# AlirezaMoseni/Distributed-Optimization-and-Learning

Measured on AMD Instinct MI355X. Metric: consensus rounds/sec at 8192 agents x 1M params (1/8 GPU) + % of HBM peak, higher is better.
Workload: dtype f32

## Files before the change

distributed-optimization-and-learning_amd/csrc/mlp_step.hip:

```cpp
#include <hip/hip_runtime.h>
#include <stdint.h>
#include <stdio.h>
#include <stdlib.h>
#include <math.h>
#include <type_traits>

#include "../../include/dol_hip.h"
#include "dol_common.h"

namespace {

typedef float f4 __attribute__((ext_vector_type(4)));
typedef float f32x16 __attribute__((ext_vector_type(16)));

constexpr int kWaves = 4;
constexpr int kThreads = 64 * kWaves;
constexpr int kMaxB = 64, kMaxH = 256, kMaxC = 32;

struct MlpArgs {
  float* W; int64_t ldw;
  float* G; int64_t ldg;
  float* M; int64_t ldm;
  const float* theta;
  const float* A; int64_t lda;
  const float* X; int64_t ldxa, ldxb;
  const int64_t* Y; int64_t ldya;
  float* loss;
  int B, d, h, c;
  float neg_lr, mom, rho;
  int mode;
  int update;
  int f1_keep;
  int dw1_reverse;
  int stagger, stagger_lo, stagger_hi, stagger_step;
#ifdef DOL_MLP_TRACE
  long long* trace;
#endif
};

#ifdef DOL_MLP_TRACE
#define DOL_TRACE(i) \
  if (threadIdx.x == 0 && a.trace) a.trace[int64_t(blockIdx.x) * 8 + (i)] = wall_clock64();
#else
#define DOL_TRACE(i)
#endif

template <int N, int UPD, bool TH, bool AL>
struct ParamBatch {
  float w[N], m[N], th[N], al[N];

  template <class Idx>
  __device__ __forceinline__ void load(const MlpArgs& a, const float* wrow, const float* mrow, const float* arow,
                                       Idx idx) {
#pragma unroll
    for (int i = 0; i < N; ++i) {
      if constexpr (UPD > 0 || TH) w[i] = wrow[idx(i)];
      if constexpr (UPD == 3) m[i] = mrow[idx(i)];
      if constexpr (TH) th[i] = a.theta[idx(i)];
      if constexpr (AL) al[i] = arow[idx(i)];
    }
  }

  template <class Idx, class Ok>
  __device__ __forceinline__ void commit(const MlpArgs& a, float* wrow, float* grow, float* mrow, const float (&g)[N],
                                         Idx idx, Ok ok) {
#pragma unroll
    for (int i = 0; i < N; ++i) {
      float gg = g[i];
      if constexpr (TH) {
        float t = a.rho * (w[i] - th[i]);
        if constexpr (AL) t = al[i] + t;
        gg = gg + t;
      }
      float dd = gg;
      if constexpr (UPD == 2) {
        m[i] = gg;
      } else if constexpr (UPD == 3) {
        m[i] = m[i] * a.mom + gg;
        dd = m[i];
      }
      if (!ok(i)) continue;
      if (grow) grow[idx(i)] = gg;
      if constexpr (UPD > 0) __builtin_nontemporal_store(__builtin_fmaf(a.neg_lr, dd, w[i]), wrow + idx(i));
      if constexpr (UPD >= 2) __builtin_nontemporal_store(m[i], mrow + idx(i));
    }
  }
};

#define DOL_GPTR(p) ((const __attribute__((address_space(1))) void*)(p))
#define DOL_LPTR(p) ((__attribute__((address_space(3))) void*)(p))

__device__ __forceinline__ void wait_vmcnt(int n) {
  switch (n) {
#define DOL_VMC(N) case N: asm volatile("s_waitcnt vmcnt(" #N ")" ::: "memory"); break;
#define DOL_VMC8(N) DOL_VMC(N) DOL_VMC(N + 1) DOL_VMC(N + 2) DOL_VMC(N + 3) DOL_VMC(N + 4) DOL_VMC(N + 5) DOL_VMC(N + 6) DOL_VMC(N + 7)
    DOL_VMC8(0) DOL_VMC8(8) DOL_VMC8(16) DOL_VMC8(24) DOL_VMC8(32) DOL_VMC8(40) DOL_VMC8(48) DOL_VMC8(56)
#undef DOL_VMC8
#undef DOL_VMC
    default: asm volatile("s_waitcnt vmcnt(0)" ::: "memory"); break;
  }
}

template <int N, class Src, class Dst>
__device__ __forceinline__ void lds_fill(int n, Src src, Dst dst) {
  const int t = threadIdx.x;
  for (int o0 = 0; o0 < n; o0 += N * kThreads) {
    float v[N];
#pragma unroll
    for (int i = 0; i < N; ++i) {
      const int o = o0 + i * kThreads + t;
      v[i] = src(o < n ? o : 0);
    }
#pragma unroll
    for (int i = 0; i < N; ++i) {
      const int o = o0 + i * kThreads + t;
      if (o < n) dst(o, v[i]);
    }
  }
}

__device__ __forceinline__ void lds_barrier() {
  asm volatile("s_waitcnt lgkmcnt(0)" ::: "memory");
  __builtin_amdgcn_s_barrier();
  asm volatile("" ::: "memory");
}

constexpr int kStages = 3;

inline int64_t fwd_union_floats(int B, int h, int c) {
  const int64_t staging = int64_t(kStages) * (h + 32 * ((B + 31) / 32)) * 32;
  const int64_t post = int64_t(B) * (h + 4) + int64_t(c) * (h + 4) + int64_t(B) * c;
  return staging > post ? staging : post;
}

using rsrc_t = __amdgpu_buffer_rsrc_t;
constexpr uint32_t kOOB = 0x80000000u;

__device__ __forceinline__ rsrc_t make_rsrc(const float* p, int64_t nbytes) {
  return __builtin_amdgcn_make_buffer_rsrc(const_cast<float*>(p), 0, static_cast<int>(nbytes), 0x00020000);
}
__device__ __forceinline__ float bload(rsrc_t r, uint32_t voff, uint32_t soff) {
  return __builtin_bit_cast(float, __builtin_amdgcn_raw_buffer_load_b32(r, static_cast<int>(voff), static_cast<int>(soff), 0));
}
__device__ __forceinline__ void bstore_nt(rsrc_t r, uint32_t voff, uint32_t soff, float v) {
  __builtin_amdgcn_raw_buffer_store_b32(__builtin_bit_cast(uint32_t, v), r, static_cast<int>(voff), static_cast<int>(soff), 2);
}

template <int NT, int UPD, bool TH, bool AL>
__device__ __forceinline__ void mlp_fwd_body(MlpArgs a, float* __restrict__ ws) {
  constexpr int NS = kStages;
  if (a.stagger > 0) {
    const int bx = int(blockIdx.x);
    if (bx >= a.stagger_lo && bx < a.stagger_hi && (bx - a.stagger_lo) % a.stagger_step == 0)
      for (int i = 0; i < a.stagger; ++i) __builtin_amdgcn_s_sleep(127);
  }
  extern __shared__ __attribute__((aligned(16))) float lds[];
  const int B = a.B, d = a.d, h = a.h, c = a.c;
  const int hp = h + 4;
  const int64_t stg_rows = h + 32 * ((B + 31) / 32);
  float* Hs = lds;
  float* W2s = Hs + B * hp;
  float* Zs = W2s + c * hp;
  const int64_t stg_f = stg_rows * (32 * NS);
  const int64_t post_f = int64_t(B) * (h + 4) + int64_t(c) * (h + 4) + int64_t(B) * c;
  float* b1s = lds + (stg_f > post_f ? stg_f : post_f);
  float* b2s = b1s + h;
  float* ls = b2s + c;
  int* ys = reinterpret_cast<int*>(ls + B);

  const int agent = blockIdx.x;
  const int t = threadIdx.x, lane = t & 63;
  const int wave = __builtin_amdgcn_readfirstlane(t >> 6);
  const int li = lane & 31, hh = lane >> 5;
  float* wrow = a.W + int64_t(agent) * a.ldw;
  float* grow = a.G ? a.G + int64_t(agent) * a.ldg : nullptr;
  float* mrow = a.M ? a.M + int64_t(agent) * a.ldm : nullptr;
  const float* arow = a.A ? a.A + int64_t(agent) * a.lda : nullptr;
  const float* xa = a.X + int64_t(agent) * a.ldxa;
  const int64_t oW1 = 0, ob1 = int64_t(h) * d, oW2 = ob1 + h, ob2 = oW2 + int64_t(c) * h;

  DOL_TRACE(0)
  auto ok_w2 = [&](int i) { return i * kThreads + t < c * h; };
  auto idx_w2 = [&](int i) { return oW2 + (ok_w2(i) ? i * kThreads + t : 0); };
  auto ok_b1 = [&](int) { return t < h; };
  auto idx_b1 = [&](int) { return ob1 + (t < h ? t : 0); };
  auto ok_b2 = [&](int) { return t < c; };
  auto idx_b2 = [&](int) { return ob2 + (t < c ? t : 0); };
  ParamBatch<8, UPD, TH, AL> pw2;
  ParamBatch<1, UPD, TH, AL> pb1, pb2;
  auto load_small = [&] {
    pw2.load(a, wrow, mrow, arow, idx_w2);
    pb1.load(a, wrow, mrow, arow, idx_b1);
    pb2.load(a, wrow, mrow, arow, idx_b2);
  };
  load_small();
  if (t < c) b2s[t] = wrow[ob2 + t];
  if (t < B) ys[t] = static_cast<int>(a.Y[int64_t(agent) * a.ldya + t]);
  for (int i = t; i < h; i += kThreads) b1s[i] = wrow[ob1 + i];
  lds_barrier();
  float* wsa = ws + int64_t(agent) * B * h;
  const bool w2_in_regs = (UPD > 0 || TH) && c * h <= 8 * kThreads;
  const int nht = h / 32, nbt = (B + 31) / 32;
  const int Bp = 32 * nbt, rows = h + Bp;
  const int ipw = rows / 32;
  const int nk = (d + 31) / 32;
  float* stg = lds;
  const rsrc_t rsX = make_rsrc(xa, (int64_t(B - 1) * a.ldxb + d) * 4);
  (void)rsX;
  auto issue = [&](int kc, const float* top, int i0) {
    float* st = stg + (kc % NS) * rows * 32;
    for (int i = i0; i < ipw; ++i) {
      const int ins = wave + kWaves * i;
      const int r = 8 * ins + (lane >> 3);
      const int ch = (lane & 7) ^ (lane >> 3);
      int k = kc * 32 + 4 * ch;
      k = k < d ? k : 0;
      const float* src = (r < h) ? top + oW1 + int64_t(r) * d + k
                                 : xa + int64_t(min(r - h, B - 1)) * a.ldxb + k;
      if (a.f1_keep)
        __builtin_amdgcn_global_load_lds(DOL_GPTR(src), DOL_LPTR(st + ins * 256), 16, 0, 0);
      else
        __builtin_amdgcn_global_load_lds(DOL_GPTR(src), DOL_LPTR(st + ins * 256), 16, 0, 2);
    }
  };
  f32x16 acc[NT];
#pragma unroll
  for (int u = 0; u < NT; ++u)
#pragma unroll
    for (int r = 0; r < 16; ++r) acc[u][r] = 0.f;
  for (int s0 = 0; s0 < NS - 1 && s0 < nk; ++s0) issue(s0, wrow, 0);
  auto f1_chunk = [&](int kc) __attribute__((always_inline)) {
    wait_vmcnt(min(NS - 2, nk - 1 - kc) * ipw);
    __builtin_amdgcn_s_barrier();
    const float* st = stg + (kc % NS) * rows * 32;
    if (kc == nk - 1 && (d & 31)) {
      for (int i = 0; i < ipw; ++i) {
        const int ins = wave + kWaves * i;
        if (kc * 32 + 4 * ((lane & 7) ^ (lane >> 3)) >= d)
          *reinterpret_cast<f4*>(const_cast<float*>(st) + ins * 256 + lane * 4) = f4{0.f, 0.f, 0.f, 0.f};
      }
      lds_barrier();
    }
    if (kc + NS - 1 < nk) issue(kc + NS - 1, wrow, 0);
#pragma unroll
    for (int u = 0; u < NT; ++u) {
      const int tile = wave + kWaves * u;
      if (tile < nht * nbt) {
        const int ht = tile % nht, bt = tile / nht;
        const float* ar = st + (32 * ht + li) * 32;
        const float* xr = st + (h + 32 * bt + li) * 32;
#pragma unroll
        for (int j = 0; j < 4; ++j) {
          const int pos = ((4 * hh + j) ^ (li & 7)) * 4;
          const f4 av = *reinterpret_cast<const f4*>(ar + pos);
          const f4 xv = *reinterpret_cast<const f4*>(xr + pos);
#pragma unroll
          for (int q = 0; q < 4; ++q) acc[u] = __builtin_amdgcn_mfma_f32_32x32x2f32(av[q], xv[q], acc[u], 0, 0, 0);
        }
      }
    }
  };
  for (int kc = 0; kc < nk; ++kc) f1_chunk(kc);
  lds_barrier();
#pragma unroll
  for (int u = 0; u < NT; ++u) {
    const int tile = wave + kWaves * u;
    if (tile < nht * nbt) {
      const int ht = tile % nht, bt = tile / nht;
      const int brow = 32 * bt + li;
      if (brow < B) {
#pragma unroll
        for (int r = 0; r < 16; ++r) {
          const int hr = 32 * ht + (r & 3) + 8 * (r >> 2) + 4 * hh;
          const float z = acc[u][r] + b1s[hr];
          Hs[brow * hp + hr] = (z > 0.0f || z != z) ? z : 0.0f;
        }
      }
    }
  }
  if (w2_in_regs) {
#pragma unroll
    for (int i = 0; i < 8; ++i)
      if (ok_w2(i)) W2s[((i * kThreads + t) / h) * hp + (i * kThreads + t) % h] = pw2.w[i];
  } else {
    lds_fill<8>(c * h, [&](int o) { return wrow[oW2 + o]; }, [&](int o, float v) { W2s[(o / h) * hp + o % h] = v; });
  }
  lds_barrier();

  DOL_TRACE(1)
  for (int o = t; o < B * c; o += kThreads) {
    const int b = o / c, j = o % c;
    float s0 = 0.0f, s1 = 0.0f, s2 = 0.0f, s3 = 0.0f;
#pragma unroll 8
    for (int k = 0; k < h; k += 4) {
      const f4 hv = *reinterpret_cast<const f4*>(Hs + b * hp + k);
      const f4 wv = *reinterpret_cast<const f4*>(W2s + j * hp + k);
      s0 = s0 + hv.x * wv.x;
      s1 = s1 + hv.y * wv.y;
      s2 = s2 + hv.z * wv.z;
      s3 = s3 + hv.w * wv.w;
    }
    Zs[o] = ((s0 + s1) + (s2 + s3)) + b2s[j];
  }
  lds_barrier();

  if (t < B) {
    float* z = Zs + t * c;
    float m = z[0];
    for (int j = 1; j < c; ++j) m = fmaxf(m, z[j]);
    float s = 0.0f;
    for (int j = 0; j < c; ++j) s = s + expf(z[j] - m);
    const float lse = m + logf(s);
    const int y = ys[t];
    const bool yok = y >= 0 && y < c;
    ls[t] = yok ? lse - z[yok ? y : 0] : __builtin_nanf("");
    const float invB = 1.0f / static_cast<float>(B);
    for (int j = 0; j < c; ++j) z[j] = (expf(z[j] - lse) - (j == y ? 1.0f : 0.0f)) * invB;
  }
  lds_barrier();
  if (t == 0 && a.loss) {
    float s = 0.0f;
#pragma unroll 8
    for (int b = 0; b < B; ++b) s = s + ls[b];
    a.loss[agent] = s / static_cast<float>(B);
  }

  DOL_TRACE(2)
  for (int o0 = 0; o0 < c * h; o0 += 8 * kThreads) {
    ParamBatch<8, UPD, TH, AL> pb;
    float g[8];
    auto ok = [&](int i) { return o0 + i * kThreads + t < c * h; };
    auto idx = [&](int i) { return oW2 + (ok(i) ? o0 + i * kThreads + t : 0); };
    if (o0 > 0) pb.load(a, wrow, mrow, arow, idx);
    if (kThreads % h == 0) {
      const int k = t % h;
      int jj[8];
#pragma unroll
      for (int i = 0; i < 8; ++i) {
        jj[i] = ok(i) ? (o0 + i * kThreads + t) / h : 0;
        g[i] = 0.0f;
      }
#pragma unroll 4
      for (int b = 0; b < B; ++b) {
        const float hv = Hs[b * hp + k];
        const float* zr = Zs + b * c;
#pragma unroll
        for (int i = 0; i < 8; ++i) g[i] = g[i] + zr[jj[i]] * hv;
      }
    } else {
#pragma unroll
      for (int i = 0; i < 8; ++i) {
        const int o = ok(i) ? o0 + i * kThreads + t : 0;
        const int j = o / h, k = o % h;
        float s = 0.0f;
        for (int b = 0; b < B; ++b) s = s + Zs[b * c + j] * Hs[b * hp + k];
        g[i] = s;
      }
    }
    if (o0 == 0) pw2.commit(a, wrow, grow, mrow, g, idx, ok);
    else pb.commit(a, wrow, grow, mrow, g, idx, ok);
  }
  DOL_TRACE(5)
  if (t < 64) {
    float g[1];
    const int j = t < c ? t : 0;
    float s = 0.0f;
#pragma unroll 8
    for (int b = 0; b < B; ++b) s = s + Zs[b * c + j];
    g[0] = s;
    pb2.commit(a, wrow, grow, mrow, g, idx_b2, ok_b2);
  }
  lds_barrier();
  DOL_TRACE(6)

  if (kThreads % h == 0 && B * h <= 16 * kThreads) {
    const int k = t % h, b0 = t / h, bs = kThreads / h;
    float sm[16];
#pragma unroll
    for (int m = 0; m < 16; ++m) sm[m] = 0.0f;
    for (int j = 0; j < c; ++j) {
      const float w2 = W2s[j * hp + k];
#pragma unroll
      for (int m = 0; m < 16; ++m) {
        const int b = b0 + m * bs;
        sm[m] = sm[m] + Zs[min(b, B - 1) * c + j] * w2;
      }
    }
#pragma unroll
    for (int m = 0; m < 16; ++m) {
      const int b = b0 + m * bs;
      if (b < B) {
        float* hv = Hs + b * hp + k;
        *hv = (*hv > 0.0f) ? sm[m] : 0.0f;
      }
    }
  } else {
#pragma unroll 4
    for (int o = t; o < B * h; o += kThreads) {
      const int b = o / h, k = o % h;
      float s = 0.0f;
      for (int j = 0; j < c; ++j) s = s + Zs[b * c + j] * W2s[j * hp + k];
      float* hv = Hs + b * hp + k;
      *hv = (*hv > 0.0f) ? s : 0.0f;
    }
  }
  lds_barrier();
  DOL_TRACE(7)

  {
    float g[1];
    float s = 0.0f;
    if (t < h)
#pragma unroll 8
      for (int b = 0; b < B; ++b) s = s + Hs[b * hp + t];
    g[0] = s;
    pb1.commit(a, wrow, grow, mrow, g, idx_b1, ok_b1);
  }

  for (int o = t; o < B * h; o += kThreads) wsa[o] = Hs[(o / h) * hp + (o % h)];
  DOL_TRACE(3)
}

template <int NT, int UPD, bool TH, bool AL>
__global__ __launch_bounds__(kThreads) void mlp_fwd_kernel(MlpArgs a, float* __restrict__ ws) {
  mlp_fwd_body<NT, UPD, TH, AL>(a, ws);
}

template <int KS, int UPD, bool TH, bool AL>
__device__ __forceinline__ void mlp_dw1_body(MlpArgs a, const float* __restrict__ ws, int n_agents) {
  const int B = a.B, d = a.d, h = a.h, c = a.c;
  const int ndt = (d + 31) / 32;
  const uint32_t bx = blockIdx.x, l = bx >> 3;
  const int dt = static_cast<int>(l % uint32_t(ndt));
  uint32_t lg = l / uint32_t(ndt);
  if (a.dw1_reverse) lg = uint32_t((n_agents + 7) / 8) - 1 - lg;
  const int agent = static_cast<int>(lg * 8 + (bx & 7));
  if (agent >= n_agents) return;
  const int lane = threadIdx.x & 63;
  const int wave = __builtin_amdgcn_readfirstlane(threadIdx.x >> 6);
  const int li = lane & 31, hh = lane >> 5;
  const int64_t P = int64_t(h) * d + h + int64_t(c) * h + c;
  const rsrc_t rW = make_rsrc(a.W + int64_t(agent) * a.ldw, P * 4);
  const rsrc_t rM = make_rsrc(UPD == 3 || UPD == 2 ? a.M + int64_t(agent) * a.ldm : a.W, P * 4);
  const rsrc_t rG = make_rsrc(a.G ? a.G + int64_t(agent) * a.ldg : a.W, a.G ? P * 4 : 0);
  const rsrc_t rT = make_rsrc(TH ? a.theta : a.W, TH ? P * 4 : 0);
  const rsrc_t rA = make_rsrc(AL ? a.A + int64_t(agent) * a.lda : a.W, AL ? P * 4 : 0);
  const rsrc_t rX = make_rsrc(a.X + int64_t(agent) * a.ldxa, (int64_t(B - 1) * a.ldxb + d) * 4);
  const rsrc_t rZ = make_rsrc(ws + int64_t(agent) * B * h, int64_t(B) * h * 4);
  const int col = 32 * dt + li;
  const bool cok = col < d;
  float xv[KS];
#pragma unroll
  for (int s = 0; s < KS; ++s) {
    const int b = 2 * s + hh;
    xv[s] = bload(rX, (b < B && cok) ? uint32_t((b * a.ldxb + col) * 4) : kOOB, 0);
  }
  for (int ht = wave; ht < h / 32; ht += kWaves) {
    float av[KS];
#pragma unroll
    for (int s = 0; s < KS; ++s) {
      const int b = 2 * s + hh;
      av[s] = bload(rZ, b < B ? uint32_t((b * h + 32 * ht + li) * 4) : kOOB, 0);
    }
    const uint32_t pv = cok ? uint32_t(((32 * ht + 4 * hh) * d + col) * 4) : kOOB;
    auto so = [&](int r) { return uint32_t(((r & 3) + 8 * (r >> 2)) * d * 4); };
    float w[16], m[16], th[16], al[16];
#pragma unroll
    for (int r = 0; r < 16; ++r) {
      if constexpr (UPD > 0 || TH) w[r] = bload(rW, pv, so(r));
      if constexpr (UPD == 3) m[r] = bload(rM, pv, so(r));
      if constexpr (TH) th[r] = bload(rT, pv, so(r));
      if constexpr (AL) al[r] = bload(rA, pv, so(r));
    }
    __builtin_amdgcn_sched_barrier(0);
    f32x16 acc;
#pragma unroll
    for (int r = 0; r < 16; ++r) acc[r] = 0.f;
    f32x16 acc1 = acc;
#pragma unroll
    for (int s = 0; s < KS; s += 2) {
      acc = __builtin_amdgcn_mfma_f32_32x32x2f32(av[s], xv[s], acc, 0, 0, 0);
      acc1 = __builtin_amdgcn_mfma_f32_32x32x2f32(av[s + 1], xv[s + 1], acc1, 0, 0, 0);
    }
    acc += acc1;
#pragma unroll
    for (int r = 0; r < 16; ++r) {
      float gg = acc[r];
      if constexpr (TH) {
        float t = a.rho * (w[r] - th[r]);
        if constexpr (AL) t = al[r] + t;
        gg = gg + t;
      }
      float dd = gg;
      if constexpr (UPD == 2) {
        m[r] = gg;
      } else if constexpr (UPD == 3) {
        m[r] = m[r] * a.mom + gg;
        dd = m[r];
      }
      if (a.G) bstore_nt(rG, pv, so(r), gg);
      if constexpr (UPD > 0) bstore_nt(rW, pv, so(r), __builtin_fmaf(a.neg_lr, dd, w[r]));
      if constexpr (UPD >= 2) bstore_nt(rM, pv, so(r), m[r]);
    }
  }
}

template <int KS, int UPD, bool TH, bool AL>
__global__ __launch_bounds__(kThreads) void mlp_dw1_kernel(MlpArgs a, const float* __restrict__ ws, int n_agents) {
  mlp_dw1_body<KS, UPD, TH, AL>(a, ws, n_agents);
}

}

extern "C" int64_t dol_mlp_step_workspace_bytes(int32_t n_agents, int32_t B, int32_t h) {
  if (n_agents <= 0 || B <= 0 || h <= 0 || B > kMaxB || h > kMaxH) return 0;
  return int64_t(n_agents) * B * h * int64_t(sizeof(float));
}

extern "C" int64_t dol_mlp_step_lds_bytes(int32_t B, int32_t h, int32_t c) {
  if (B <= 0 || h <= 0 || c <= 0 || B > kMaxB || h > kMaxH || c > kMaxC) return 0;
  return sizeof(float) * (fwd_union_floats(B, h, c) + h + c + B) + sizeof(int) * int64_t(B);
}

extern "C" int dol_mlp_step_f32(float* w, int64_t ldw, float* grad, int64_t ldg, float* mom, int64_t ldm,
                                const float* theta, const float* alpha, int64_t lda, const float* X,
                                int64_t ldx_agent, int64_t ldx_row, const int64_t* labels, int64_t ldy_agent,
                                float* loss, int32_t n_agents, int32_t B, int32_t d, int32_t h, int32_t c,
                                float lr, float momentum, float rho, int first_step, int update,
                                void* work, hipStream_t s) {
  DOL_DIMS_OK("dol_mlp_step_f32", ldw, ldg, ldm, lda, ldx_agent, ldx_row, ldy_agent);
  using dol::fail;
  if (n_agents < 0) return fail(DOL_EINVAL, "dol_mlp_step_f32: negative agent count");
  if (n_agents == 0) { dol::g_err[0] = '\0'; return DOL_OK; }
  if (B < 1 || B > kMaxB) return fail(DOL_EINVAL, "dol_mlp_step_f32: batch %d outside [1, %d]", B, kMaxB);
  if (h < 32 || h > kMaxH || h % 32) return fail(DOL_EINVAL, "dol_mlp_step_f32: hidden %d must be a multiple of 32 in [32, %d]", h, kMaxH);
  if (c < 1 || c > kMaxC) return fail(DOL_EINVAL, "dol_mlp_step_f32: classes %d outside [1, %d]", c, kMaxC);
  if (d < 4 || d % 4) return fail(DOL_EINVAL, "dol_mlp_step_f32: input dim %d must be a positive multiple of 4", d);
  if (!w || !X || !labels || !work) return fail(DOL_EINVAL, "dol_mlp_step_f32: null w / X / labels / work");
  const int64_t P = int64_t(h) * d + h + int64_t(c) * h + c;
  if (ldw < P || (grad && ldg < P) || (mom && ldm < P) || (alpha && lda < P))
    return fail(DOL_EINVAL, "dol_mlp_step_f32: ld < P (%lld)", (long long)P);
  if (ldx_row < d || ldx_agent < int64_t(B - 1) * ldx_row + d || ldy_agent < B)
    return fail(DOL_EINVAL, "dol_mlp_step_f32: X / labels strides too small");
  if ((reinterpret_cast<uintptr_t>(w) & 15) || ldw % 4 || (reinterpret_cast<uintptr_t>(X) & 15) || ldx_row % 4 ||
      ldx_agent % 4)
    return fail(DOL_EINVAL, "dol_mlp_step_f32: w and X rows must be 16-byte aligned");
  if (alpha && !theta) return fail(DOL_EINVAL, "dol_mlp_step_f32: alpha without theta");
  const int mode = (momentum == 0.0f) ? 0 : (first_step ? 1 : 2);
  if (update && mode != 0 && !mom) return fail(DOL_EINVAL, "dol_mlp_step_f32: momentum needs the mom buffer");
  if (!update && !grad) return fail(DOL_EINVAL, "dol_mlp_step_f32: update=0 needs a grad buffer to write");
  MlpArgs a{w, ldw, grad, ldg, mom, ldm, theta, alpha, lda, X, ldx_agent, ldx_row, labels, ldy_agent, loss,
            B, d, h, c, -lr, momentum, rho, update ? mode : 0, update ? 1 : 0};
  static const int f1_keep = [] { const char* e = getenv("DOL_MLP_F1_KEEP"); return e ? atoi(e) : 1; }();
  static const int dw1_rev = [] { const char* e = getenv("DOL_MLP_DW1_REVERSE"); return e ? atoi(e) : 1; }();
  a.f1_keep = f1_keep;
  a.dw1_reverse = dw1_rev;
  {
    static const int n_cu = [] {
      int dev = 0, cu = 0;
      if (hipGetDevice(&dev) != hipSuccess ||
          hipDeviceGetAttribute(&cu, hipDeviceAttributeMultiprocessorCount, dev) != hipSuccess)
        cu = 0;
      return cu;
    }();
    const char* e = getenv("DOL_MLP_FWD_STAGGER");
    int cnt = (n_cu > 0 && n_agents >= 4 * n_cu) ? 6 : 0, mode = 1;
    if (e && sscanf(e, "%d,%d", &cnt, &mode) < 1) cnt = 0;
    if (cnt > 0 && n_cu > 0) {
      a.stagger = cnt;
      a.stagger_lo = mode == 2 ? 1 : n_cu;
      a.stagger_hi = 2 * n_cu;
      a.stagger_step = mode == 2 ? 2 : 1;
    }
  }
  const size_t lds = static_cast<size_t>(dol_mlp_step_lds_bytes(B, h, c));
  if (lds > 160 * 1024) return fail(DOL_EINVAL, "dol_mlp_step_f32: %zu B of LDS per agent exceeds 160 KiB", lds);
  const dim3 grid(static_cast<unsigned>(n_agents)), block(kThreads);
  const int upd = update ? mode + 1 : 0;
  float* ws = static_cast<float*>(work);
  const int64_t n_blk2 = int64_t((d + 31) / 32) * ((int64_t(n_agents) + 7) / 8 * 8);
  if (n_blk2 > (int64_t(1) << 31) - 1) return fail(DOL_EINVAL, "dol_mlp_step_f32: too many W1 tiles for one launch");
  const dim3 grid2(static_cast<unsigned>(n_blk2));
  auto go = [&](auto ks, auto upd_c, auto th, auto al) {
    constexpr int KS = decltype(ks)::value, U = decltype(upd_c)::value;
    constexpr bool TH = decltype(th)::value, AL = decltype(al)::value;
    auto fwd = [&](auto kern) {
      if (lds > 65536)
        (void)hipFuncSetAttribute(reinterpret_cast<const void*>(kern), hipFuncAttributeMaxDynamicSharedMemorySize,
                                  static_cast<int>(lds));
      hipLaunchKernelGGL(kern, grid, block, lds, s, a, ws);
    };
    if (h * ((B + 31) / 32) <= 128) fwd(mlp_fwd_kernel<1, U, TH, AL>);
    else fwd(mlp_fwd_kernel<4, U, TH, AL>);
    hipLaunchKernelGGL((mlp_dw1_kernel<KS, U, TH, AL>), grid2, block, 0, s, a, ws, n_agents);
  };
  auto by_upd = [&](auto ks, auto th, auto al) {
    using std::integral_constant;
    switch (upd) {
      case 0: go(ks, integral_constant<int, 0>{}, th, al); break;
      case 1: go(ks, integral_constant<int, 1>{}, th, al); break;
      case 2: go(ks, integral_constant<int, 2>{}, th, al); break;
      default: go(ks, integral_constant<int, 3>{}, th, al); break;
    }
  };
  using K16 = std::integral_constant<int, 16>;
  using K32 = std::integral_constant<int, 32>;
  using T = std::true_type;
  using F = std::false_type;
  if (B <= 32) {
    if (!theta) by_upd(K16{}, F{}, F{});
    else if (!alpha) by_upd(K16{}, T{}, F{});
    else by_upd(K16{}, T{}, T{});
  } else {
    if (!theta) by_upd(K32{}, F{}, F{});
    else if (!alpha) by_upd(K32{}, T{}, F{});
    else by_upd(K32{}, T{}, T{});
  }
  return dol::check_launch("dol_mlp_step_f32");
}
```

Baseline: 92.62.

## Move MLP second-layer forward and backward matmuls onto MFMA 32x32x2 f32

Replaces the scalar LDS dot-product loops for the layer-2 logits, the W2 gradient and the hidden-layer backprop with MFMA 32x32x2 f32 tiles split across waves. Per-wave partial logits go to a new LDS scratch buffer, and a separate pass reduces them and computes the softmax with wave shuffles instead of one thread per row. The W2 gradient and dH are computed in one fused pass, with the workspace write merged into it. LDS buffers are padded to 32 rows/classes, which increases LDS use and may lower occupancy. The code assumes c<=32 and B<=64.

```diff
diff --git a/distributed-optimization-and-learning_amd/csrc/mlp_step.hip b/distributed-optimization-and-learning_amd/csrc/mlp_step.hip
--- a/distributed-optimization-and-learning_amd/csrc/mlp_step.hip
+++ b/distributed-optimization-and-learning_amd/csrc/mlp_step.hip
@@ -127,9 +127,14 @@
 
 constexpr int kStages = 3;
 
+constexpr int kCp = 32;
+constexpr int kZp = 33;
+
 inline int64_t fwd_union_floats(int B, int h, int c) {
-  const int64_t staging = int64_t(kStages) * (h + 32 * ((B + 31) / 32)) * 32;
-  const int64_t post = int64_t(B) * (h + 4) + int64_t(c) * (h + 4) + int64_t(B) * c;
+  (void)c;
+  const int64_t Bp = 32 * ((B + 31) / 32);
+  const int64_t staging = int64_t(kStages) * (h + Bp) * 32;
+  const int64_t post = Bp * (h + 4) + int64_t(kCp) * (h + 4) + Bp * kZp + int64_t(kWaves) * Bp * 32;
   return staging > post ? staging : post;
 }
 
@@ -158,11 +163,14 @@
   const int B = a.B, d = a.d, h = a.h, c = a.c;
   const int hp = h + 4;
   const int64_t stg_rows = h + 32 * ((B + 31) / 32);
+  const int Bpad = 32 * ((B + 31) / 32);
   float* Hs = lds;
-  float* W2s = Hs + B * hp;
-  float* Zs = W2s + c * hp;
+  float* W2s = Hs + Bpad * hp;
+  float* Zs = W2s + kCp * hp;
+  float* Ps = Zs + Bpad * kZp;
   const int64_t stg_f = stg_rows * (32 * NS);
-  const int64_t post_f = int64_t(B) * (h + 4) + int64_t(c) * (h + 4) + int64_t(B) * c;
+  const int64_t post_f = int64_t(Bpad) * (h + 4) + int64_t(kCp) * (h + 4) + int64_t(Bpad) * kZp +
+                         int64_t(kWaves) * Bpad * 32;
   float* b1s = lds + (stg_f > post_f ? stg_f : post_f);
   float* b2s = b1s + h;
   float* ls = b2s + c;
@@ -285,128 +293,152 @@
   } else {
     lds_fill<8>(c * h, [&](int o) { return wrow[oW2 + o]; }, [&](int o, float v) { W2s[(o / h) * hp + o % h] = v; });
   }
+  for (int o = B * hp + t; o < Bpad * hp; o += kThreads) Hs[o] = 0.0f;
+  for (int o = c * hp + t; o < kCp * hp; o += kThreads) W2s[o] = 0.0f;
   lds_barrier();
 
   DOL_TRACE(1)
-  for (int o = t; o < B * c; o += kThreads) {
-    const int b = o / c, j = o % c;
-    float s0 = 0.0f, s1 = 0.0f, s2 = 0.0f, s3 = 0.0f;
-#pragma unroll 8
-    for (int k = 0; k < h; k += 4) {
-      const f4 hv = *reinterpret_cast<const f4*>(Hs + b * hp + k);
-      const f4 wv = *reinterpret_cast<const f4*>(W2s + j * hp + k);
-      s0 = s0 + hv.x * wv.x;
-      s1 = s1 + hv.y * wv.y;
-      s2 = s2 + hv.z * wv.z;
-      s3 = s3 + hv.w * wv.w;
-    }
-    Zs[o] = ((s0 + s1) + (s2 + s3)) + b2s[j];
+  auto rrow = [&](int r) { return (r & 3) + 8 * (r >> 2) + 4 * hh; };
+  {
+    f32x16 z2[2];
+#pragma unroll
+    for (int bt = 0; bt < 2; ++bt)
+#pragma unroll
+      for (int r = 0; r < 16; ++r) z2[bt][r] = 0.f;
+    for (int ht = wave; ht < nht; ht += kWaves) {
+      const int k0 = 32 * ht + 4 * hh;
+#pragma unroll
+      for (int jj = 0; jj < 4; ++jj) {
+        const f4 wv = *reinterpret_cast<const f4*>(W2s + li * hp + k0 + 8 * jj);
+#pragma unroll
+        for (int bt = 0; bt < 2; ++bt) {
+          if (bt < nbt) {
+            const f4 hv = *reinterpret_cast<const f4*>(Hs + (32 * bt + li) * hp + k0 + 8 * jj);
+#pragma unroll
+            for (int q = 0; q < 4; ++q) z2[bt] = __builtin_amdgcn_mfma_f32_32x32x2f32(hv[q], wv[q], z2[bt], 0, 0, 0);
+          }
+        }
+      }
+    }
+#pragma unroll
+    for (int bt = 0; bt < 2; ++bt)
+      if (bt < nbt)
+#pragma unroll
+        for (int r = 0; r < 16; ++r) Ps[(wave * Bpad + 32 * bt + rrow(r)) * 32 + li] = z2[bt][r];
   }
   lds_barrier();
 
-  if (t < B) {
-    float* z = Zs + t * c;
-    float m = z[0];
-    for (int j = 1; j < c; ++j) m = fmaxf(m, z[j]);
-    float s = 0.0f;
-    for (int j = 0; j < c; ++j) s = s + expf(z[j] - m);
-    const float lse = m + logf(s);
-    const int y = ys[t];
-    const bool yok = y >= 0 && y < c;
-    ls[t] = yok ? lse - z[yok ? y : 0] : __builtin_nanf("");
+  {
     const float invB = 1.0f / static_cast<float>(B);
-    for (int j = 0; j < c; ++j) z[j] = (expf(z[j] - lse) - (j == y ? 1.0f : 0.0f)) * invB;
+    const int tile = Bpad * 32;
+    for (int o = t; o < tile; o += kThreads) {
+      const int b = o >> 5, j = o & 31;
+      const bool live = j < c, bok = b < B;
+      float z = ((Ps[o] + Ps[tile + o]) + Ps[2 * tile + o]) + Ps[3 * tile + o];
+      z = z + b2s[live ? j : 0];
+      float m = live ? z : -INFINITY;
+#pragma unroll
+      for (int x = 16; x > 0; x >>= 1) m = fmaxf(m, __shfl_xor(m, x));
+      float s = live ? expf(z - m) : 0.0f;
+#pragma unroll
+      for (int x = 16; x > 0; x >>= 1) s = s + __shfl_xor(s, x);
+      const float lse = m + logf(s);
+      const int y = ys[bok ? b : B - 1];
+      const bool yok = y >= 0 && y < c;
+      const float zy = __shfl(z, (lane & 32) | (yok ? y : 0));
+      if (j == 0 && bok) ls[b] = yok ? lse - zy : __builtin_nanf("");
+      Zs[b * kZp + j] = (live && bok) ? (expf(z - lse) - (j == y ? 1.0f : 0.0f)) * invB : 0.0f;
+    }
   }
   lds_barrier();
-  if (t == 0 && a.loss) {
-    float s = 0.0f;
-#pragma unroll 8
-    for (int b = 0; b < B; ++b) s = s + ls[b];
-    a.loss[agent] = s / static_cast<float>(B);
-  }
 
   DOL_TRACE(2)
-  for (int o0 = 0; o0 < c * h; o0 += 8 * kThreads) {
-    ParamBatch<8, UPD, TH, AL> pb;
-    float g[8];
-    auto ok = [&](int i) { return o0 + i * kThreads + t < c * h; };
-    auto idx = [&](int i) { return oW2 + (ok(i) ? o0 + i * kThreads + t : 0); };
-    if (o0 > 0) pb.load(a, wrow, mrow, arow, idx);
-    if (kThreads % h == 0) {
-      const int k = t % h;
-      int jj[8];
+  {
+    const int nsb = (B + 1) / 2, nsc = (c + 1) / 2;
+    for (int ht = wave; ht < nht; ht += kWaves) {
+      const int kcol = 32 * ht + li;
+      f32x16 gw, dz[2];
+#pragma unroll
+      for (int r = 0; r < 16; ++r) gw[r] = dz[0][r] = dz[1][r] = 0.f;
+      for (int s0 = 0; s0 < nsb; s0 += 8) {
+        float za[8], hb[8];
+#pragma unroll
+        for (int u = 0; u < 8; ++u) {
+          za[u] = Zs[(2 * (s0 + u) + hh) * kZp + li];
+          hb[u] = Hs[(2 * (s0 + u) + hh) * hp + kcol];
+        }
+#pragma unroll
+        for (int u = 0; u < 8; ++u) gw = __builtin_amdgcn_mfma_f32_32x32x2f32(za[u], hb[u], gw, 0, 0, 0);
+      }
+      for (int s0 = 0; s0 < nsc; s0 += 4) {
+        float w2[4], za[2][4];
+#pragma unroll
+        for (int u = 0; u < 4; ++u) {
+          w2[u] = W2s[(2 * (s0 + u) + hh) * hp + kcol];
+#pragma unroll
+          for (int bt = 0; bt < 2; ++bt) za[bt][u] = Zs[(32 * (bt < nbt ? bt : 0) + li) * kZp + 2 * (s0 + u) + hh];
+        }
+#pragma unroll
+        for (int u = 0; u < 4; ++u)
+#pragma unroll
+          for (int bt = 0; bt < 2; ++bt)
+            if (bt < nbt) dz[bt] = __builtin_amdgcn_mfma_f32_32x32x2f32(za[bt][u], w2[u], dz[bt], 0, 0, 0);
+      }
+#pragma unroll
+      for (int bt = 0; bt < 2; ++bt) {
+        if (bt < nbt) {
+#pragma unroll
+          for (int r = 0; r < 16; ++r) {
+            const int b = 32 * bt + rrow(r);
+            if (b < B) {
+              float* hv = Hs + b * hp + kcol;
+              const float v = (*hv > 0.0f) ? dz[bt][r] : 0.0f;
+              *hv = v;
+              wsa[b * h + kcol] = v;
+            }
+          }
+        }
+      }
+#pragma unroll
+      for (int r = 0; r < 16; ++r) W2s[rrow(r) * hp + kcol] = gw[r];
+    }
+  }
+  lds_barrier();
+  DOL_TRACE(5)
+
+  {
+    const int dj = kThreads / h, dk = kThreads % h;
+    int j = t / h, k = t % h;
+    for (int o0 = 0; o0 < c * h; o0 += 8 * kThreads) {
+      ParamBatch<8, UPD, TH, AL> pb;
+      float g[8];
+      auto ok = [&](int i) { return o0 + i * kThreads + t < c * h; };
+      auto idx = [&](int i) { return oW2 + (ok(i) ? o0 + i * kThreads + t : 0); };
+      if (o0 > 0) pb.load(a, wrow, mrow, arow, idx);
 #pragma unroll
       for (int i = 0; i < 8; ++i) {
-        jj[i] = ok(i) ? (o0 + i * kThreads + t) / h : 0;
-        g[i] = 0.0f;
-      }
-#pragma unroll 4
-      for (int b = 0; b < B; ++b) {
-        const float hv = Hs[b * hp + k];
-        const float* zr = Zs + b * c;
-#pragma unroll
-        for (int i = 0; i < 8; ++i) g[i] = g[i] + zr[jj[i]] * hv;
-      }
-    } else {
-#pragma unroll
-      for (int i = 0; i < 8; ++i) {
-        const int o = ok(i) ? o0 + i * kThreads + t : 0;
-        const int j = o / h, k = o % h;
-        float s = 0.0f;
-        for (int b = 0; b < B; ++b) s = s + Zs[b * c + j] * Hs[b * hp + k];
-        g[i] = s;
-      }
-    }
-    if (o0 == 0) pw2.commit(a, wrow, grow, mrow, g, idx, ok);
-    else pb.commit(a, wrow, grow, mrow, g, idx, ok);
-  }
-  DOL_TRACE(5)
+        g[i] = W2s[min(j, kCp - 1) * hp + k];
+        j += dj;
+        k += dk;
+        if (k >= h) {
+          k -= h;
+          ++j;
+        }
+      }
+      if (o0 == 0) pw2.commit(a, wrow, grow, mrow, g, idx, ok);
+      else pb.commit(a, wrow, grow, mrow, g, idx, ok);
+    }
+  }
+  DOL_TRACE(6)
   if (t < 64) {
     float g[1];
     const int j = t < c ? t : 0;
     float s = 0.0f;
 #pragma unroll 8
-    for (int b = 0; b < B; ++b) s = s + Zs[b * c + j];
+    for (int b = 0; b < B; ++b) s = s + Zs[b * kZp + j];
     g[0] = s;
     pb2.commit(a, wrow, grow, mrow, g, idx_b2, ok_b2);
   }
-  lds_barrier();
-  DOL_TRACE(6)
-
-  if (kThreads % h == 0 && B * h <= 16 * kThreads) {
-    const int k = t % h, b0 = t / h, bs = kThreads / h;
-    float sm[16];
-#pragma unroll
-    for (int m = 0; m < 16; ++m) sm[m] = 0.0f;
-    for (int j = 0; j < c; ++j) {
-      const float w2 = W2s[j * hp + k];
-#pragma unroll
-      for (int m = 0; m < 16; ++m) {
-        const int b = b0 + m * bs;
-        sm[m] = sm[m] + Zs[min(b, B - 1) * c + j] * w2;
-      }
-    }
-#pragma unroll
-    for (int m = 0; m < 16; ++m) {
-      const int b = b0 + m * bs;
-      if (b < B) {
-        float* hv = Hs + b * hp + k;
-        *hv = (*hv > 0.0f) ? sm[m] : 0.0f;
-      }
-    }
-  } else {
-#pragma unroll 4
-    for (int o = t; o < B * h; o += kThreads) {
-      const int b = o / h, k = o % h;
-      float s = 0.0f;
-      for (int j = 0; j < c; ++j) s = s + Zs[b * c + j] * W2s[j * hp + k];
-      float* hv = Hs + b * hp + k;
-      *hv = (*hv > 0.0f) ? s : 0.0f;
-    }
-  }
-  lds_barrier();
-  DOL_TRACE(7)
-
   {
     float g[1];
     float s = 0.0f;
@@ -416,8 +448,13 @@
     g[0] = s;
     pb1.commit(a, wrow, grow, mrow, g, idx_b1, ok_b1);
   }
-
-  for (int o = t; o < B * h; o += kThreads) wsa[o] = Hs[(o / h) * hp + (o % h)];
+  DOL_TRACE(7)
+  if (t == kThreads - 64 && a.loss) {
+    float s = 0.0f;
+#pragma unroll 8
+    for (int b = 0; b < B; ++b) s = s + ls[b];
+    a.loss[agent] = s / static_cast<float>(B);
+  }
   DOL_TRACE(3)
 }
 
```

New measurement: 92.62, median of 3. Within noise of the previous version (-0.0%).
